# 0xPolygonZero/plonky2

Measured on NVIDIA H100. Metric: goldilocks_field_elements_per_s_ntt_lde_merkle, higher is better.
Workload: dtype u64

## Files before the change

plonky2_b200/csrc/gl_lazy.cuh:

```cuda
#pragma once
#include "gl_field.cuh"

namespace gl {

struct L3 {
    uint32_t w0, w1;
    int32_t e;
};

GL_HD L3 l3_from(uint64_t x) { return L3{(uint32_t)x, (uint32_t)(x >> 32), 0}; }

#if defined(__CUDA_ARCH__)
__device__ __forceinline__ L3 l3_add(L3 a, L3 b) {
    L3 r;
    asm("add.cc.u32 %0, %3, %6;\n\taddc.cc.u32 %1, %4, %7;\n\taddc.u32 %2, %5, %8;"
        : "=r"(r.w0), "=r"(r.w1), "=r"(r.e)
        : "r"(a.w0), "r"(a.w1), "r"(a.e), "r"(b.w0), "r"(b.w1), "r"(b.e));
    return r;
}
__device__ __forceinline__ L3 l3_sub(L3 a, L3 b) {
    L3 r;
    asm("sub.cc.u32 %0, %3, %6;\n\tsubc.cc.u32 %1, %4, %7;\n\tsubc.u32 %2, %5, %8;"
        : "=r"(r.w0), "=r"(r.w1), "=r"(r.e)
        : "r"(a.w0), "r"(a.w1), "r"(a.e), "r"(b.w0), "r"(b.w1), "r"(b.e));
    return r;
}
template <int S>
__device__ __forceinline__ L3 l3_shift(L3 a) {
    static_assert(S >= 0 && S < 96, "shift out of range");
    if constexpr (S == 0) return a;
    constexpr int q = S / 32, r = S % 32;
    uint32_t c0, c1, c2;
    int32_t c3;
    if constexpr (r == 0) {
        c0 = a.w0;
        c1 = a.w1;
        c2 = (uint32_t)a.e;
        c3 = a.e >> 31;
    } else {
        c0 = a.w0 << r;
        c1 = __funnelshift_l(a.w0, a.w1, r);
        c2 = __funnelshift_l(a.w1, (uint32_t)a.e, r);
        c3 = a.e >> (32 - r);
    }
    const int32_t s3 = c3 >> 31;
    L3 o;
    if (q == 0) {
        uint32_t t0, t1, b1, be;
        asm("add.cc.u32 %0, %2, %3;\n\taddc.u32 %1, %4, 0;" : "=r"(t0), "=r"(t1) : "r"(c2), "r"((uint32_t)c3), "r"((uint32_t)s3));
        asm("add.cc.u32 %0, %2, %3;\n\taddc.u32 %1, 0, 0;" : "=r"(b1), "=r"(be) : "r"(c1), "r"(c2));
        asm("sub.cc.u32 %0, %3, %5;\n\tsubc.cc.u32 %1, %4, %6;\n\tsubc.u32 %2, %7, %8;"
            : "=r"(o.w0), "=r"(o.w1), "=r"(o.e)
            : "r"(c0), "r"(b1), "r"(t0), "r"(t1), "r"(be), "r"((int32_t)t1 >> 31));
    } else if (q == 1) {
        uint32_t b1, be, t0, t1;
        int32_t t2;
        asm("add.cc.u32 %0, %2, %3;\n\taddc.u32 %1, 0, 0;" : "=r"(b1), "=r"(be) : "r"(c0), "r"(c1));
        asm("add.cc.u32 %0, %3, %4;\n\taddc.cc.u32 %1, %5, 0;\n\taddc.u32 %2, %6, 0;"
            : "=r"(t0), "=r"(t1), "=r"(t2)
            : "r"(c1), "r"(c2), "r"((uint32_t)c3), "r"(s3));
        asm("sub.cc.u32 %0, 0, %3;\n\tsubc.cc.u32 %1, %4, %5;\n\tsubc.u32 %2, %6, %7;"
            : "=r"(o.w0), "=r"(o.w1), "=r"(o.e)
            : "r"(t0), "r"(b1), "r"(t1), "r"(be), "r"(t2));
    } else {
        uint32_t u0, u1, v0, v1, t1;
        int32_t t2;
        asm("add.cc.u32 %0, %2, %3;\n\taddc.u32 %1, 0, 0;" : "=r"(u0), "=r"(u1) : "r"(c0), "r"(c1));
        asm("sub.cc.u32 %0, %0, %2;\n\tsubc.u32 %1, %1, %3;" : "+r"(u0), "+r"(u1) : "r"((uint32_t)c3), "r"((uint32_t)s3));
        asm("add.cc.u32 %0, %2, %3;\n\taddc.u32 %1, %4, 0;" : "=r"(v0), "=r"(v1) : "r"(c2), "r"((uint32_t)c3), "r"((uint32_t)s3));
        asm("add.cc.u32 %0, %2, %3;\n\taddc.u32 %1, %4, %5;" : "=r"(t1), "=r"(t2) : "r"(u1), "r"(v0), "r"((int32_t)u1 >> 31), "r"(v1));
        asm("sub.cc.u32 %0, 0, %3;\n\tsubc.cc.u32 %1, %4, %5;\n\tsubc.u32 %2, 0, %6;"
            : "=r"(o.w0), "=r"(o.w1), "=r"(o.e)
            : "r"(u0), "r"(c0), "r"(t1), "r"(t2));
    }
    return o;
}
__device__ __forceinline__ uint64_t l3_norm(L3 a) {
    uint32_t w0, w1, e;
    asm("add.cc.u32 %0, %3, 0x00100000;\n\taddc.cc.u32 %1, %4, 0xfff00000;\n\taddc.u32 %2, %5, 0x000fffff;"
        : "=r"(w0), "=r"(w1), "=r"(e)
        : "r"(a.w0), "r"(a.w1), "r"(a.e));
    return reduce96(pack64(w0, w1), e);
}
#else
inline __int128 l3_val(L3 a) { return (__int128)a.w0 + ((__int128)a.w1 << 32) + (__int128)a.e * ((__int128)1 << 64); }
inline L3 l3_of(__int128 v) {
    L3 r;
    r.w0 = (uint32_t)(unsigned __int128)v;
    r.w1 = (uint32_t)((unsigned __int128)v >> 32);
    r.e = (int32_t)(v >> 64);
    return r;
}
inline L3 l3_add(L3 a, L3 b) { return l3_of(l3_val(a) + l3_val(b)); }
inline L3 l3_sub(L3 a, L3 b) { return l3_of(l3_val(a) - l3_val(b)); }
inline uint64_t l3_norm(L3 a) {
    __int128 v = l3_val(a) % (__int128)P;
    if (v < 0) v += P;
    return (uint64_t)v;
}
template <int S>
inline L3 l3_shift(L3 a) { return l3_from(mul_pow2(l3_norm(a), (uint32_t)S)); }
#endif

template <int S>
GL_HD L3 l3_shift_c(L3 a) { return l3_shift<S>(a); }
template <int M, int L, int B>
struct DftLazyBfly {
    static GL_HD void run(L3* r) {
        constexpr int half = 1 << (M - 1 - L);
        constexpr int j = B % half, blk = (B / half) * 2 * half;
        constexpr int sh = (96 / half) * j;
        const L3 u = r[blk + j], v = r[blk + j + half];
        r[blk + j] = l3_add(u, v);
        r[blk + j + half] = l3_shift_c<sh>(l3_sub(u, v));
        if constexpr (B + 1 < (1 << (M - 1))) DftLazyBfly<M, L, B + 1>::run(r);
        else if constexpr (L + 1 < M) DftLazyBfly<M, L + 1, 0>::run(r);
    }
};
template <int M>
GL_HD void dft_lazy(L3* r) {
    if constexpr (M > 0) DftLazyBfly<M, 0, 0>::run(r);
}

}
```

plonky2_b200/csrc/gl_ntt.cuh:

```cuda
#pragma once
#include "gl_lazy.cuh"

namespace gl {

constexpr int NTT_MAX_LOG_PASS = 10;
constexpr int NTT_COL_MIN_LOG = 5;

GL_HD constexpr int ntt_r2(int log) { return log / 2; }
GL_HD constexpr int ntt_r1(int log) { return log - log / 2; }

template <int LOG>
struct PassCfg {
    static constexpr int R1 = ntt_r1(LOG), R2 = ntt_r2(LOG);
    static constexpr int E = 1 << R1, TPT = 1 << R2, NSUB = E / TPT;
    static constexpr int ROW_THREADS = (TPT * 8 < 32) ? 32 : TPT * 8;
    static constexpr int LPC = ROW_THREADS / TPT;
    static constexpr int ROW_MIN_BLOCKS = (E >= 32 ? 512 : 768) / ROW_THREADS;
    static constexpr int ROW_PITCH = TPT + 1;
    static constexpr int ROW_S_WORDS = E * ROW_PITCH;
    static constexpr int GATHER_PITCH = (1 << LOG) + 2;
    static constexpr int T = (256 / TPT) < 8 ? 8 : (256 / TPT);
    static constexpr int COL_THREADS = T * TPT;
    static constexpr int COL_MIN_BLOCKS = (E >= 32 ? 512 : 768) / COL_THREADS;
    static constexpr int COL_QPITCH = TPT * T + 8;
    static constexpr int COL_S_WORDS = E * COL_QPITCH;
};
GL_HD constexpr size_t ntt_row_smem_bytes(int log, bool natural) {
    const int r1 = ntt_r1(log), r2 = ntt_r2(log), E = 1 << r1, TPT = 1 << r2;
    const int threads = (TPT * 8 < 32) ? 32 : TPT * 8, lpc = threads / TPT;
    const size_t s = (size_t)lpc * E * (TPT + 1), g = natural ? (size_t)lpc * ((1 << log) + 2) : 0;
    return (s > g ? s : g) * 8;
}
GL_HD constexpr size_t ntt_col_smem_bytes(int log) {
    const int r1 = ntt_r1(log), r2 = ntt_r2(log), E = 1 << r1, TPT = 1 << r2;
    const int T = (256 / TPT) < 8 ? 8 : (256 / TPT);
    return (size_t)E * (TPT * T + 8) * 8;
}

GL_HD uint64_t table_step_entry(int log, uint32_t idx, uint64_t scale, uint64_t base) {
    const int r1 = ntt_r1(log), r2 = ntt_r2(log);
    const uint32_t t = idx & ((1u << r2) - 1), q = idx >> r2;
    const uint64_t k = bitrev32(q, (uint32_t)r1);
    uint64_t v = pow(root_of_unity((uint32_t)log), k * t);
    if (base != 1) v = mul(v, pow(base, t));
    if (scale != 1) v = mul(v, scale);
    return v;
}
GL_HD uint64_t table_post_entry(int a, int b, size_t idx, uint64_t base) {
    const size_t p = idx >> b, j2 = idx & (((size_t)1 << b) - 1);
    const uint64_t k1 = bitrev32((uint32_t)p, (uint32_t)a);
    uint64_t v = pow(root_of_unity((uint32_t)(a + b)), k1 * j2);
    if (base != 1) v = mul(v, pow(base, j2));
    return v;
}

template <int LOG>
GL_HD void pass_step1(uint64_t* x, const uint64_t* tw, const uint64_t* uq, bool tw_full, int t) {
    using Cf = PassCfg<LOG>;
    L3 r[Cf::E];
#pragma unroll
    for (int q = 0; q < Cf::E; q++) {
        uint64_t v = x[q];
        if (uq && q) v = mul(v, uq[q]);
        r[q] = l3_from(v);
    }
    dft_lazy<Cf::R1>(r);
#pragma unroll
    for (int q = 0; q < Cf::E; q++) {
        uint64_t y = l3_norm(r[q]);
        if (Cf::R2 > 0 && (q || tw_full)) y = mul(y, tw[q * Cf::TPT + t]);
        if (Cf::R2 == 0 && tw_full) y = mul(y, tw[0]);
        x[q] = y;
    }
}
template <int LOG>
GL_HD void pass_step2(uint64_t* z) {
    using Cf = PassCfg<LOG>;
    L3 r[Cf::TPT];
#pragma unroll
    for (int j = 0; j < Cf::TPT; j++) r[j] = l3_from(z[j]);
    dft_lazy<Cf::R2>(r);
#pragma unroll
    for (int j = 0; j < Cf::TPT; j++) z[j] = l3_norm(r[j]);
}

struct ColPass {
    const uint64_t* in;
    uint64_t* out;
    size_t in_stride, out_stride;
    const uint64_t* tw;
    const uint64_t* twa;
    int log_c;
    int log_rb;
    int tw_full;
    int has_uq;
    uint64_t uq[32];
};
template <int LOG>
GL_HD void col_unit(const ColPass& cp, int blk, size_t& in_off, size_t& out_off, int& tile) {
    using Cf = PassCfg<LOG>;
    const int tiles = (1 << cp.log_c) / Cf::T;
    tile = blk % tiles;
    const int unit = blk / tiles;
    const size_t rb = (size_t)unit & (((size_t)1 << cp.log_rb) - 1), col = (size_t)unit >> cp.log_rb;
    const size_t blk_words = (size_t)1 << (LOG + cp.log_c);
    in_off = col * cp.in_stride + rb * blk_words;
    out_off = col * cp.out_stride + rb * blk_words;
}
template <int LOG>
GL_HD void col_load(const ColPass& cp, int blk, int tid, uint64_t* x) {
    using Cf = PassCfg<LOG>;
    const int tt = tid % Cf::T, t = tid / Cf::T;
    size_t in_off, out_off;
    int tile;
    col_unit<LOG>(cp, blk, in_off, out_off, tile);
    const size_t C = (size_t)1 << cp.log_c;
    const uint64_t* src = cp.in + in_off + (size_t)tile * Cf::T + tt;
#pragma unroll
    for (int q = 0; q < Cf::E; q++) x[q] = src[(size_t)(t + Cf::TPT * q) * C];
}
template <int LOG>
GL_HD void col_phase1(const ColPass& cp, uint64_t* S, int blk, int tid, uint64_t* x) {
    using Cf = PassCfg<LOG>;
    const int tt = tid % Cf::T, t = tid / Cf::T;
    size_t in_off, out_off;
    int tile;
    col_unit<LOG>(cp, blk, in_off, out_off, tile);
    const size_t C = (size_t)1 << cp.log_c;
    pass_step1<LOG>(x, cp.tw, cp.has_uq ? cp.uq : nullptr, cp.tw_full != 0, t);
    if (Cf::R2 == 0) {
        uint64_t* dst = cp.out + out_off + (size_t)tile * Cf::T + tt;
        const uint64_t* twa = cp.twa + (size_t)tile * Cf::T + tt;
#pragma unroll
        for (int q = 0; q < Cf::E; q++) dst[(size_t)q * C] = mul(x[q], twa[(size_t)q * C]);
        return;
    }
#pragma unroll
    for (int q = 0; q < Cf::E; q++) S[q * Cf::COL_QPITCH + t * Cf::T + tt] = x[q];
}
template <int LOG>
GL_HD void col_phase2_load(const uint64_t* S, int tid, uint64_t* z ) {
    using Cf = PassCfg<LOG>;
    const int tt = tid % Cf::T, t = tid / Cf::T;
#pragma unroll
    for (int m = 0; m < Cf::NSUB; m++) {
        const int q = t + Cf::TPT * m;
#pragma unroll
        for (int j = 0; j < Cf::TPT; j++) z[m * Cf::TPT + j] = S[q * Cf::COL_QPITCH + j * Cf::T + tt];
    }
}
template <int LOG>
GL_HD void col_phase2_dft(uint64_t* z) {
    using Cf = PassCfg<LOG>;
#pragma unroll
    for (int m = 0; m < Cf::NSUB; m++) pass_step2<LOG>(z + m * Cf::TPT);
}
template <int LOG>
GL_HD int col_twiddle_slot(int tid, int i) { return i * PassCfg<LOG>::COL_THREADS + tid; }
template <int LOG>
GL_HD const uint64_t* col_twiddle_src(const ColPass& cp, int blk, int tid, int i) {
    using Cf = PassCfg<LOG>;
    const int tt = tid % Cf::T, t = tid / Cf::T;
    size_t in_off, out_off;
    int tile;
    col_unit<LOG>(cp, blk, in_off, out_off, tile);
    const int m = i / Cf::TPT, j = i % Cf::TPT;
    const size_t p = (size_t)(t + Cf::TPT * m) * Cf::TPT + j;
    return cp.twa + (p << cp.log_c) + (size_t)tile * Cf::T + tt;
}
template <int LOG>
GL_HD void col_phase2_store(const ColPass& cp, int blk, int tid, const uint64_t* z, const uint64_t* tws, size_t stride_j,
                            size_t stride_m) {
    using Cf = PassCfg<LOG>;
    const int tt = tid % Cf::T, t = tid / Cf::T;
    size_t in_off, out_off;
    int tile;
    col_unit<LOG>(cp, blk, in_off, out_off, tile);
    const size_t C = (size_t)1 << cp.log_c;
    uint64_t* dst = cp.out + out_off + (size_t)tile * Cf::T + tt;
#pragma unroll
    for (int m = 0; m < Cf::NSUB; m++) {
#pragma unroll
        for (int j = 0; j < Cf::TPT; j++) {
            const int i = m * Cf::TPT + j;
            const size_t p = (size_t)(t + Cf::TPT * m) * Cf::TPT + j;
            dst[p * C] = mul(z[i], tws[m * stride_m + j * stride_j]);
        }
    }
}
template <int LOG>
GL_HD void col_phase2(const ColPass& cp, const uint64_t* S, int blk, int tid) {
    using Cf = PassCfg<LOG>;
    if (Cf::R2 == 0) return;
    uint64_t z[Cf::E];
    col_phase2_load<LOG>(S, tid, z);
    col_phase2_dft<LOG>(z);
    const size_t C = (size_t)1 << cp.log_c;
    col_phase2_store<LOG>(cp, blk, tid, z, col_twiddle_src<LOG>(cp, blk, tid, 0), C, (size_t)Cf::TPT * Cf::TPT * C);
}

enum RowMode { RM_BITREV = 0, RM_NATURAL = 1 };
struct RowPass {
    const uint64_t* in;
    uint64_t* out;
    size_t in_stride, out_stride;
    const uint64_t* tw;
    int log_r;
    int ncols;
    int tw_full;
    int has_uq;
    int reverse;
    size_t row0;
    int n_peer;
    uint64_t* out_peer[7];
    uint64_t uq[32];
};
template <int LOG, int MODE>
GL_HD bool row_line(const RowPass& rp, int blk, int l, size_t& col, size_t& prow, size_t& kbase) {
    using Cf = PassCfg<LOG>;
    const size_t L = (size_t)blk * Cf::LPC + l;
    const size_t R = (size_t)1 << rp.log_r;
    col = L >> rp.log_r;
    const size_t low = L & (R - 1);
    if (MODE == RM_BITREV) {
        prow = low;
        kbase = 0;
    } else {
        kbase = low;
        prow = rp.log_r ? (size_t)bitrev32((uint32_t)low, (uint32_t)rp.log_r) : 0;
    }
    return col < (size_t)rp.ncols;
}
template <int LOG>
GL_HD int row_blocks(const RowPass& rp) {
    using Cf = PassCfg<LOG>;
    const size_t lines = (size_t)rp.ncols << rp.log_r;
    return (int)((lines + Cf::LPC - 1) / Cf::LPC);
}
template <int LOG, int MODE>
GL_HD void row_load(const RowPass& rp, int blk, int tid, uint64_t* x) {
    using Cf = PassCfg<LOG>;
    const int l = tid / Cf::TPT, t = tid % Cf::TPT;
    size_t col, prow, kbase;
    const bool live = row_line<LOG, MODE>(rp, blk, l, col, prow, kbase);
    const uint64_t* src = rp.in + col * rp.in_stride + (prow << LOG) + t;
#pragma unroll
    for (int q = 0; q < Cf::E; q++) x[q] = live ? src[Cf::TPT * q] : 0;
}
template <int LOG, int MODE>
GL_HD void row_phase1(const RowPass& rp, uint64_t* S, int blk, int tid, uint64_t* x) {
    using Cf = PassCfg<LOG>;
    const int l = tid / Cf::TPT, t = tid % Cf::TPT;
    pass_step1<LOG>(x, rp.tw, rp.has_uq ? rp.uq : nullptr, rp.tw_full != 0, t);
    if (Cf::R2 == 0) return;
    uint64_t* Sl = S + (size_t)l * Cf::ROW_S_WORDS;
#pragma unroll
    for (int q = 0; q < Cf::E; q++) Sl[q * Cf::ROW_PITCH + t] = x[q];
}
template <int LOG>
GL_HD uint32_t row_natural_index(int q, int j) {
    using Cf = PassCfg<LOG>;
    return bitrev32((uint32_t)q, Cf::R1) + (uint32_t)Cf::E * (Cf::R2 ? bitrev32((uint32_t)j, Cf::R2) : 0u);
}
template <int LOG>
GL_HD void row_phase2_load(const uint64_t* S, int tid, int m, uint64_t* z) {
    using Cf = PassCfg<LOG>;
    const int l = tid / Cf::TPT, t = tid % Cf::TPT;
    const uint64_t* Sl = S + (size_t)l * Cf::ROW_S_WORDS;
    const int q = t + Cf::TPT * m;
#pragma unroll
    for (int j = 0; j < Cf::TPT; j++) z[j] = Sl[q * Cf::ROW_PITCH + j];
}
template <int LOG>
GL_HD void row_store_bitrev(const RowPass& rp, int blk, int tid, int m, const uint64_t* z) {
    using Cf = PassCfg<LOG>;
    const int l = tid / Cf::TPT, t = tid % Cf::TPT;
    size_t col, prow, kbase;
    if (!row_line<LOG, RM_BITREV>(rp, blk, l, col, prow, kbase)) return;
    uint64_t* dst = rp.out + col * rp.out_stride + rp.row0 + (prow << LOG);
    if constexpr (Cf::R2 == 0) {
#pragma unroll
        for (int q = 0; q < Cf::E; q++) dst[q] = canon(z[q]);
    } else {
        const int q = t + Cf::TPT * m;
        uint64_t* d = dst + (size_t)q * Cf::TPT;
#if defined(__CUDA_ARCH__)
#pragma unroll
        for (int j = 0; j < Cf::TPT; j += 2) {
            ulonglong2 v;
            v.x = canon(z[j]);
            v.y = canon(z[j + 1]);
            *reinterpret_cast<ulonglong2*>(d + j) = v;
        }
#else
        for (int j = 0; j < Cf::TPT; j++) d[j] = canon(z[j]);
#endif
    }
}
template <int LOG>
GL_HD void row_gather_write(uint64_t* G, int tid, int m, const uint64_t* z) {
    using Cf = PassCfg<LOG>;
    const int l = tid / Cf::TPT, t = tid % Cf::TPT;
    uint64_t* Gl = G + (size_t)l * Cf::GATHER_PITCH;
    if (Cf::R2 == 0) {
#pragma unroll
        for (int q = 0; q < Cf::E; q++) Gl[row_natural_index<LOG>(q, 0)] = canon(z[q]);
        return;
    }
    const int q = t + Cf::TPT * m;
#pragma unroll
    for (int j = 0; j < Cf::TPT; j++) Gl[row_natural_index<LOG>(q, j)] = canon(z[j]);
}
template <int LOG>
GL_HD void row_store_natural(const RowPass& rp, const uint64_t* G, int blk, int tid, int nthreads) {
    using Cf = PassCfg<LOG>;
    const size_t R = (size_t)1 << rp.log_r, n = R << LOG;
    for (int e = tid; e < Cf::LPC * (1 << LOG); e += nthreads) {
        int l, k2;
        if (rp.log_r) {
            l = e % Cf::LPC;
            k2 = e / Cf::LPC;
        } else {
            k2 = e & ((1 << LOG) - 1);
            l = e >> LOG;
        }
        size_t col, prow, kbase;
        if (!row_line<LOG, RM_NATURAL>(rp, blk, l, col, prow, kbase)) continue;
        size_t k = kbase + ((size_t)k2 << rp.log_r);
        if (rp.reverse) k = (n - k) & (n - 1);
        const uint64_t v = G[(size_t)l * Cf::GATHER_PITCH + k2];
        const size_t at = col * rp.out_stride + k;
        rp.out[at] = v;
        for (int p = 0; p < rp.n_peer; p++) rp.out_peer[p][at] = v;
    }
}

struct NttPlan {
    int a1, a2, b;
};
GL_HD NttPlan ntt_plan(int log_n) {
    NttPlan p{0, 0, log_n};
    if (log_n <= NTT_MAX_LOG_PASS) return p;
    if (log_n <= 2 * NTT_MAX_LOG_PASS) {
        p.b = (log_n + 1) / 2;
        p.a1 = log_n - p.b;
        return p;
    }
    p.b = (log_n + 2) / 3;
    p.a2 = (log_n - p.b + 1) / 2;
    p.a1 = log_n - p.b - p.a2;
    return p;
}


struct TableReq {
    int a, b;
    uint64_t scale, base;
};
struct NttJob {
    NttPlan pl;
    ColPass c1, c2;
    RowPass rp;
    TableReq c1_step, c1_post, c2_step, c2_post, row_step;
};
inline void ntt_make_job(int log_n, NttPlan pl, uint64_t scale, uint64_t shift, NttJob& job) {
    job = NttJob{};
    job.pl = pl;
    const bool coset = canon(shift) != 1;
    const uint64_t one = 1;
    RowPass& rp = job.rp;
    rp.log_r = log_n - pl.b;
    auto fill_uq = [](uint64_t* uq, int log_pass, uint64_t sq) {
        const int E = 1 << ntt_r1(log_pass);
        uint64_t acc = 1;
        for (int q = 0; q < E; q++, acc = mul(acc, sq)) uq[q] = canon(acc);
    };
    if (pl.a1 == 0) {
        job.row_step = TableReq{pl.b, 0, scale, coset ? shift : one};
        rp.tw_full = (canon(scale) != 1 || coset) ? 1 : 0;
        rp.has_uq = coset ? 1 : 0;
        if (coset) fill_uq(rp.uq, pl.b, pow(shift, (uint64_t)1 << ntt_r2(pl.b)));
        return;
    }
    const int c1_log = log_n - pl.a1;
    ColPass& c1 = job.c1;
    c1.log_c = c1_log;
    c1.log_rb = 0;
    job.c1_step = TableReq{pl.a1, 0, one, coset ? pow(shift, (uint64_t)1 << c1_log) : one};
    job.c1_post = TableReq{pl.a1, c1_log, one, coset ? shift : one};
    c1.tw_full = coset ? 1 : 0;
    c1.has_uq = coset ? 1 : 0;
    if (coset) fill_uq(c1.uq, pl.a1, pow(shift, ((uint64_t)1 << ntt_r2(pl.a1)) << c1_log));
    if (pl.a2) {
        ColPass& c2 = job.c2;
        c2.log_c = pl.b;
        c2.log_rb = pl.a1;
        job.c2_step = TableReq{pl.a2, 0, one, one};
        job.c2_post = TableReq{pl.a2, pl.b, one, one};
    }
    job.row_step = TableReq{pl.b, 0, scale, one};
    rp.tw_full = canon(scale) != 1 ? 1 : 0;
}
template <int LOG>
GL_HD int col_blocks(const ColPass& cp, size_t ncols) {
    return (int)((ncols << cp.log_rb) * (((size_t)1 << cp.log_c) / PassCfg<LOG>::T));
}

}
```

plonky2_b200/csrc/gl_ntt_host.cuh:

```cuda
#pragma once

template <int LOG, bool ASYNC_TW>
__global__ void __launch_bounds__(PassCfg<LOG>::COL_THREADS, PassCfg<LOG>::COL_MIN_BLOCKS) k_ntt_col(ColPass cp) {
    using Cf = PassCfg<LOG>;
    extern __shared__ __align__(16) u64 smem[];
    u64* tw_s = smem;
    u64* S = smem + (1 << LOG);
    u64* mbar = S + Cf::COL_S_WORDS;
    tma_table_issue(tw_s, cp.tw, (uint32_t)((1 << LOG) * 8), mbar);
    u64 x[Cf::E];
    col_load<LOG>(cp, blockIdx.x, threadIdx.x, x);
    __syncthreads();
    ColPass c2 = cp;
    c2.tw = tw_s;
    tma_table_wait(mbar);
    col_phase1<LOG>(c2, S, blockIdx.x, threadIdx.x, x);
    if (Cf::R2 == 0) return;
    __syncthreads();
    if (!ASYNC_TW) {
        col_phase2<LOG>(c2, S, blockIdx.x, threadIdx.x);
        return;
    }
    col_phase2_load<LOG>(S, threadIdx.x, x);
    __syncthreads();
#pragma unroll
    for (int i = 0; i < Cf::E; i++) {
        const u64* src = col_twiddle_src<LOG>(cp, blockIdx.x, threadIdx.x, i);
        asm volatile("cp.async.ca.shared.global [%0], [%1], 8;" ::"r"(smem_u32(S + col_twiddle_slot<LOG>(threadIdx.x, i))), "l"(src)
                     : "memory");
    }
    asm volatile("cp.async.commit_group;" ::: "memory");
    col_phase2_dft<LOG>(x);
    asm volatile("cp.async.wait_group 0;" ::: "memory");
    col_phase2_store<LOG>(cp, blockIdx.x, threadIdx.x, x, S + col_twiddle_slot<LOG>(threadIdx.x, 0), Cf::COL_THREADS,
                          (size_t)Cf::TPT * Cf::COL_THREADS);
}

template <int LOG, bool ASYNC_TW>
__global__ void __launch_bounds__(PassCfg<LOG>::COL_THREADS, PassCfg<LOG>::COL_MIN_BLOCKS) k_ntt_col_shared(ColPass cp) {
    using Cf = PassCfg<LOG>;
    static_assert(Cf::E == Cf::TPT, "shared-body column pass needs an even LOG");
    extern __shared__ __align__(16) u64 smem[];
    u64* tw_s = smem;
    u64* S = smem + (1 << LOG);
    u64* mbar = S + Cf::COL_S_WORDS;
    tma_table_issue(tw_s, cp.tw, (uint32_t)((1 << LOG) * 8), mbar);
    u64 x[Cf::E];
    col_load<LOG>(cp, blockIdx.x, threadIdx.x, x);
    __syncthreads();
    tma_table_wait(mbar);
    const int tt = threadIdx.x % Cf::T, t = threadIdx.x / Cf::T;
    size_t in_off, out_off;
    int tile;
    col_unit<LOG>(cp, blockIdx.x, in_off, out_off, tile);
    const size_t C = (size_t)1 << cp.log_c;
    if (cp.has_uq) {
#pragma unroll
        for (int q = 1; q < Cf::E; q++) x[q] = mul(x[q], cp.uq[q]);
    }
    const u64* twp = tw_s + t;
    size_t tws = Cf::TPT;
    bool skip0 = cp.tw_full == 0;
#pragma unroll 1
    for (int s = 0; s < 2; s++) {
        L3 r[Cf::E];
#pragma unroll
        for (int q = 0; q < Cf::E; q++) r[q] = l3_from(x[q]);
        dft_lazy<Cf::R1>(r);
        if (ASYNC_TW && s == 1) asm volatile("cp.async.wait_group 0;" ::: "memory");
#pragma unroll
        for (int q = 0; q < Cf::E; q++) {
            u64 y = l3_norm(r[q]);
            if (!(q == 0 && skip0)) y = mul(y, twp[(size_t)q * tws]);
            x[q] = y;
        }
        if (s == 0) {
#pragma unroll
            for (int q = 0; q < Cf::E; q++) S[q * Cf::COL_QPITCH + t * Cf::T + tt] = x[q];
            __syncthreads();
#pragma unroll
            for (int j = 0; j < Cf::TPT; j++) x[j] = S[t * Cf::COL_QPITCH + j * Cf::T + tt];
            skip0 = false;
            const u64* tw2 = cp.twa + (((size_t)t * Cf::TPT) << cp.log_c) + (size_t)tile * Cf::T + tt;
            if (ASYNC_TW) {
                __syncthreads();
#pragma unroll
                for (int j = 0; j < Cf::TPT; j++)
                    asm volatile("cp.async.ca.shared.global [%0], [%1], 8;" ::"r"(smem_u32(S + col_twiddle_slot<LOG>(threadIdx.x, j))),
                                 "l"(tw2 + (size_t)j * C)
                                 : "memory");
                asm volatile("cp.async.commit_group;" ::: "memory");
                twp = S + col_twiddle_slot<LOG>(threadIdx.x, 0);
                tws = Cf::COL_THREADS;
            } else {
                twp = tw2;
                tws = C;
            }
        }
    }
    u64* dst = cp.out + out_off + (size_t)tile * Cf::T + tt;
#pragma unroll
    for (int j = 0; j < Cf::TPT; j++) dst[((size_t)t * Cf::TPT + j) * C] = x[j];
}

template <int LOG, int MODE>
__global__ void __launch_bounds__(PassCfg<LOG>::ROW_THREADS, PassCfg<LOG>::ROW_MIN_BLOCKS) k_ntt_row(RowPass rp) {
    using Cf = PassCfg<LOG>;
    extern __shared__ __align__(16) u64 smem[];
    u64* tw_s = smem;
    u64* S = smem + (1 << LOG);
    u64* mbar = S + ntt_row_smem_bytes(LOG, MODE == RM_NATURAL) / 8;
    RowPass r2 = rp;
    u64 x[Cf::E];
    if (Cf::R2 > 0 && LOG >= 4) {
        tma_table_issue(tw_s, rp.tw, (uint32_t)((1 << LOG) * 8), mbar);
        row_load<LOG, MODE>(rp, blockIdx.x, threadIdx.x, x);
        __syncthreads();
        r2.tw = tw_s;
        tma_table_wait(mbar);
    } else {
        row_load<LOG, MODE>(rp, blockIdx.x, threadIdx.x, x);
    }
    row_phase1<LOG, MODE>(r2, S, blockIdx.x, threadIdx.x, x);
    if (Cf::R2 == 0) {
        if (MODE == RM_BITREV) {
            row_store_bitrev<LOG>(r2, blockIdx.x, threadIdx.x, 0, x);
        } else {
            row_gather_write<LOG>(S, threadIdx.x, 0, x);
            __syncthreads();
            row_store_natural<LOG>(r2, S, blockIdx.x, threadIdx.x, blockDim.x);
        }
        return;
    }
    __syncwarp();
    if (MODE == RM_BITREV) {
#pragma unroll
        for (int m = 0; m < Cf::NSUB; m++) {
            u64 z[Cf::TPT];
            row_phase2_load<LOG>(S, threadIdx.x, m, z);
            pass_step2<LOG>(z);
            row_store_bitrev<LOG>(r2, blockIdx.x, threadIdx.x, m, z);
        }
    } else {
        u64 z[Cf::NSUB][Cf::TPT];
#pragma unroll
        for (int m = 0; m < Cf::NSUB; m++) {
            row_phase2_load<LOG>(S, threadIdx.x, m, z[m]);
            pass_step2<LOG>(z[m]);
        }
        __syncthreads();
#pragma unroll
        for (int m = 0; m < Cf::NSUB; m++) row_gather_write<LOG>(S, threadIdx.x, m, z[m]);
        __syncthreads();
        row_store_natural<LOG>(r2, S, blockIdx.x, threadIdx.x, blockDim.x);
    }
}

template <int LOG, int MODE>
__global__ void __launch_bounds__(PassCfg<LOG>::ROW_THREADS, PassCfg<LOG>::ROW_MIN_BLOCKS) k_ntt_row_shared(RowPass rp) {
    using Cf = PassCfg<LOG>;
    static_assert(Cf::E == Cf::TPT && Cf::R2 > 0 && LOG >= 4, "shared-body row pass needs an even LOG >= 4");
    extern __shared__ __align__(16) u64 smem[];
    u64* tw_s = smem;
    u64* S = smem + (1 << LOG);
    u64* mbar = S + ntt_row_smem_bytes(LOG, MODE == RM_NATURAL) / 8;
    u64 x[Cf::E];
    tma_table_issue(tw_s, rp.tw, (uint32_t)((1 << LOG) * 8), mbar);
    row_load<LOG, MODE>(rp, blockIdx.x, threadIdx.x, x);
    __syncthreads();
    tma_table_wait(mbar);
    const int l = threadIdx.x / Cf::TPT, t = threadIdx.x % Cf::TPT;
    u64* Sl = S + (size_t)l * Cf::ROW_S_WORDS;
    if (rp.has_uq) {
#pragma unroll
        for (int q = 1; q < Cf::E; q++) x[q] = mul(x[q], rp.uq[q]);
    }
    const bool skip0 = rp.tw_full == 0;
    bool do_mul = true;
#pragma unroll 1
    for (int s = 0; s < 2; s++) {
        L3 r[Cf::E];
#pragma unroll
        for (int q = 0; q < Cf::E; q++) r[q] = l3_from(x[q]);
        dft_lazy<Cf::R1>(r);
#pragma unroll
        for (int q = 0; q < Cf::E; q++) {
            u64 y = l3_norm(r[q]);
            if (do_mul && !(q == 0 && skip0)) y = mul(y, tw_s[q * Cf::TPT + t]);
            x[q] = y;
        }
        if (s == 0) {
#pragma unroll
            for (int q = 0; q < Cf::E; q++) Sl[q * Cf::ROW_PITCH + t] = x[q];
            __syncwarp();
#pragma unroll
            for (int j = 0; j < Cf::TPT; j++) x[j] = Sl[t * Cf::ROW_PITCH + j];
            do_mul = false;
        }
    }
    if (MODE == RM_BITREV) {
        row_store_bitrev<LOG>(rp, blockIdx.x, threadIdx.x, 0, x);
    } else {
        __syncthreads();
        row_gather_write<LOG>(S, threadIdx.x, 0, x);
        __syncthreads();
        row_store_natural<LOG>(rp, S, blockIdx.x, threadIdx.x, blockDim.x);
    }
}

__global__ void k_fill_step(int log, u64 scale, u64 base, u64* out) {
    uint32_t j = blockIdx.x * blockDim.x + threadIdx.x;
    if (j < (1u << log)) out[j] = table_step_entry(log, j, scale, base);
}
__global__ void k_fill_post(int a, int b, u64 base, u64* out) {
    size_t i = (size_t)blockIdx.x * blockDim.x + threadIdx.x;
    if (i < ((size_t)1 << (a + b))) out[i] = table_post_entry(a, b, i, base);
}
__global__ void k_fill_pows(const u64* bases, int ntab, size_t count, u64* out) {
    size_t i = (size_t)blockIdx.x * blockDim.x + threadIdx.x;
    if (i >= count * ntab) return;
    size_t t = i / count, e = i % count;
    out[i] = gl::pow(bases[t], e);
}
__global__ void k_mul_pows(u64* data, size_t stride, size_t n, const u64* hi, const u64* lo, int lowbits) {
    size_t k = (size_t)blockIdx.x * blockDim.x + threadIdx.x;
    if (k >= n) return;
    u64* col = data + (size_t)blockIdx.y * stride;
    u64 f = mul(hi[k >> lowbits], lo[k & (((size_t)1 << lowbits) - 1)]);
    col[k] = canon(mul(col[k], f));
}

template <int LOG>
static int launch_col(gl_ctx* ctx, const ColPass& cp, size_t ncols) {
    const int nblocks = col_blocks<LOG>(cp, ncols);
    const size_t smem = ((size_t)(1 << LOG) + PassCfg<LOG>::COL_S_WORDS) * 8 + 16;
    auto go = [&](auto kern) -> int {
        const void* fn = (const void*)kern;
        if (!ctx->smem_attr_done.count(fn)) {
            CK(ctx, cudaFuncSetAttribute(kern, cudaFuncAttributeMaxDynamicSharedMemorySize, (int)smem));
            CK(ctx, cudaFuncSetAttribute(kern, cudaFuncAttributePreferredSharedMemoryCarveout, cudaSharedmemCarveoutMaxShared));
            ctx->smem_attr_done.insert(fn);
        }
        kern<<<nblocks, PassCfg<LOG>::COL_THREADS, smem, ctx->stream>>>(cp);
        CKL(ctx);
        return GL_OK;
    };
    if constexpr (PassCfg<LOG>::E == PassCfg<LOG>::TPT) {
        if (ctx->ntt_variant == 0) return cp.has_uq ? go(k_ntt_col_shared<LOG, true>) : go(k_ntt_col_shared<LOG, false>);
    }
    return cp.has_uq ? go(k_ntt_col<LOG, true>) : go(k_ntt_col<LOG, false>);
}
template <int LOG, int MODE>
static int launch_row(gl_ctx* ctx, const RowPass& rp) {
    const size_t smem = (size_t)(1 << LOG) * 8 + ntt_row_smem_bytes(LOG, MODE == RM_NATURAL) + 16;
    auto go = [&](auto kern) -> int {
        const void* fn = (const void*)kern;
        if (!ctx->smem_attr_done.count(fn)) {
            CK(ctx, cudaFuncSetAttribute(kern, cudaFuncAttributeMaxDynamicSharedMemorySize, (int)smem));
            CK(ctx, cudaFuncSetAttribute(kern, cudaFuncAttributePreferredSharedMemoryCarveout, cudaSharedmemCarveoutMaxShared));
            ctx->smem_attr_done.insert(fn);
        }
        kern<<<row_blocks<LOG>(rp), PassCfg<LOG>::ROW_THREADS, smem, ctx->stream>>>(rp);
        CKL(ctx);
        return GL_OK;
    };
    if constexpr (PassCfg<LOG>::E == PassCfg<LOG>::TPT && LOG >= 4) {
        if (ctx->ntt_variant == 0) return go(k_ntt_row_shared<LOG, MODE>);
    }
    return go(k_ntt_row<LOG, MODE>);
}
static int dispatch_col(gl_ctx* ctx, int a, const ColPass& cp, size_t ncols) {
    switch (a) {
        case 5: return launch_col<5>(ctx, cp, ncols);
        case 6: return launch_col<6>(ctx, cp, ncols);
        case 7: return launch_col<7>(ctx, cp, ncols);
        case 8: return launch_col<8>(ctx, cp, ncols);
        case 9: return launch_col<9>(ctx, cp, ncols);
        case 10: return launch_col<10>(ctx, cp, ncols);
    }
    return set_err(ctx, GL_ERR_UNSUPPORTED, "column pass log %d", a);
}
static int dispatch_row(gl_ctx* ctx, int b, int mode, const RowPass& rp) {
#define ROW_CASE(L)                                                     \
    case L:                                                             \
        return mode == RM_BITREV ? launch_row<L, RM_BITREV>(ctx, rp) : launch_row<L, RM_NATURAL>(ctx, rp);
    switch (b) {
        ROW_CASE(1) ROW_CASE(2) ROW_CASE(3) ROW_CASE(4) ROW_CASE(5) ROW_CASE(6) ROW_CASE(7) ROW_CASE(8) ROW_CASE(9) ROW_CASE(10)
    }
#undef ROW_CASE
    return set_err(ctx, GL_ERR_UNSUPPORTED, "row pass log %d", b);
}

static void table_cache_trim(gl_ctx* ctx, size_t incoming_bytes) {
    const size_t cap = (size_t)3 << 30;
    if (ctx->table_bytes + incoming_bytes <= cap) return;
    for (auto& kv : ctx->step_tabs) cudaFreeAsync(kv.second, ctx->stream);
    for (auto& kv : ctx->post_tabs) cudaFreeAsync(kv.second, ctx->stream);
    ctx->step_tabs.clear();
    ctx->post_tabs.clear();
    ctx->table_bytes = 0;
}
static int get_step(gl_ctx* ctx, int log, u64 scale, u64 base, const u64** out) {
    auto key = std::make_tuple(log, canon(scale), canon(base));
    auto it = ctx->step_tabs.find(key);
    if (it == ctx->step_tabs.end()) {
        const size_t words = ((size_t)1 << log) < 2 ? 2 : ((size_t)1 << log);
        DevBuf p(ctx);
        TRY(p.alloc(words));
        k_fill_step<<<((1 << log) + 255) / 256, 256, 0, ctx->stream>>>(log, canon(scale), canon(base), p.get());
        CKL(ctx);
        ctx->table_bytes += words * 8;
        it = ctx->step_tabs.emplace(key, p.release()).first;
    }
    *out = it->second;
    return GL_OK;
}
static int get_post(gl_ctx* ctx, int a, int b, u64 base, const u64** out) {
    auto key = std::make_tuple(a, b, canon(base));
    auto it = ctx->post_tabs.find(key);
    if (it == ctx->post_tabs.end()) {
        const size_t words = (size_t)1 << (a + b);
        DevBuf p(ctx);
        TRY(p.alloc(words));
        k_fill_post<<<(unsigned)((words + 255) / 256), 256, 0, ctx->stream>>>(a, b, canon(base), p.get());
        CKL(ctx);
        ctx->table_bytes += words * 8;
        it = ctx->post_tabs.emplace(key, p.release()).first;
    }
    *out = it->second;
    return GL_OK;
}
static uint32_t group_cols(const gl_ctx* ctx, int log_n, uint32_t ncols) {
    uint32_t g = ctx->ntt_group;
    if (g == 0) {
        size_t col_bytes = (size_t)8 << log_n;
        size_t target = (size_t)1 << 30;
        g = (uint32_t)(target / col_bytes);
        if (g < 8) g = 8;
    }
    g = (g + 7) & ~7u;
    if (g > ((ncols + 7) & ~7u)) g = (ncols + 7) & ~7u;
    return g;
}

static int build_pow_tables(gl_ctx* ctx, const std::vector<u64>& bases, size_t count, DevBuf& out) {
    const int ntab = (int)bases.size();
    DevBuf dbases(ctx);
    TRY(dbases.alloc(ntab));
    TRY(h2d(ctx, dbases.get(), bases.data(), ntab));
    TRY(out.alloc(count * ntab));
    size_t total = count * ntab;
    k_fill_pows<<<(unsigned)((total + 255) / 256), 256, 0, ctx->stream>>>(dbases.get(), ntab, count, out.get());
    CKL(ctx);
    return GL_OK;
}

struct PeerOuts {
    int n = 0;
    u64* p[7] = {nullptr, nullptr, nullptr, nullptr, nullptr, nullptr, nullptr};
};
static int ntt_forward(gl_ctx* ctx, const u64* in, size_t in_stride, u64* out, size_t out_stride, size_t row0, int log_n,
                       uint32_t ncols, int mode, bool reverse, u64 scale, u64 shift, const PeerOuts* peers = nullptr) {
    if (ncols == 0) return GL_OK;
    if (log_n < 1 || log_n > 3 * NTT_MAX_LOG_PASS) return set_err(ctx, GL_ERR_UNSUPPORTED, "log_n %d not in 1..30", log_n);
    const NttPlan pl = ntt_plan(log_n);
    const size_t n = (size_t)1 << log_n;
    table_cache_trim(ctx, 2 * n * 8 + (1 << 16));
    NttJob job;
    ntt_make_job(log_n, pl, scale, shift, job);
    RowPass& rp = job.rp;
    rp.out_stride = out_stride;
    rp.reverse = reverse ? 1 : 0;
    rp.row0 = row0;
    rp.n_peer = peers ? peers->n : 0;
    for (int i = 0; i < rp.n_peer; i++) rp.out_peer[i] = peers->p[i];
    TRY(get_step(ctx, job.row_step.a, job.row_step.scale, job.row_step.base, &rp.tw));
    if (pl.a1 == 0) {
        rp.in = in;
        rp.in_stride = in_stride;
        rp.out = out;
        rp.ncols = (int)ncols;
        return dispatch_row(ctx, pl.b, mode, rp);
    }
    const uint32_t G = group_cols(ctx, log_n, ncols);
    TRY(ensure_scratch(ctx, (size_t)G * n));
    ColPass &c1 = job.c1, &c2 = job.c2;
    c1.out = ctx->scratch;
    c1.in_stride = in_stride;
    c1.out_stride = n;
    TRY(get_step(ctx, job.c1_step.a, job.c1_step.scale, job.c1_step.base, &c1.tw));
    TRY(get_post(ctx, job.c1_post.a, job.c1_post.b, job.c1_post.base, &c1.twa));
    if (pl.a2) {
        c2.in = c2.out = ctx->scratch;
        c2.in_stride = c2.out_stride = n;
        TRY(get_step(ctx, job.c2_step.a, job.c2_step.scale, job.c2_step.base, &c2.tw));
        TRY(get_post(ctx, job.c2_post.a, job.c2_post.b, job.c2_post.base, &c2.twa));
    }
    rp.in = ctx->scratch;
    rp.in_stride = n;
    for (uint32_t g0 = 0; g0 < ncols; g0 += G) {
        const uint32_t gc = (ncols - g0 < G) ? ncols - g0 : G;
        c1.in = in + (size_t)g0 * in_stride;
        TRY(dispatch_col(ctx, pl.a1, c1, gc));
        if (pl.a2) TRY(dispatch_col(ctx, pl.a2, c2, gc));
        rp.out = out + (size_t)g0 * out_stride;
        for (int i = 0; i < rp.n_peer; i++) rp.out_peer[i] = peers->p[i] + (size_t)g0 * out_stride;
        rp.ncols = (int)gc;
        TRY(dispatch_row(ctx, pl.b, mode, rp));
    }
    return GL_OK;
}

__global__ void k_scale1(u64* data, size_t stride, uint32_t ncols, u64 f) {
    uint32_t b = blockIdx.x * blockDim.x + threadIdx.x;
    if (b < ncols) data[(size_t)b * stride] = canon(mul(data[(size_t)b * stride], f));
}

static int ntt_natural(gl_ctx* ctx, const u64* in, size_t in_stride, u64* out, size_t out_stride, int log_n,
                       uint32_t ncols, bool inverse, u64 shift, const PeerOuts* peers = nullptr) {
    if (ncols == 0) return GL_OK;
    const size_t n = (size_t)1 << log_n;
    if (peers && peers->n && (log_n == 0 || canon(shift) != 1))
        return set_err(ctx, GL_ERR_UNSUPPORTED, "multi-destination transforms need log_n >= 1 and no coset shift");
    if (log_n == 0) {
        if (in != out)
            CK(ctx, cudaMemcpy2DAsync(out, out_stride * 8, in, in_stride * 8, 8, ncols, cudaMemcpyDeviceToDevice,
                                      ctx->stream));
        k_scale1<<<(ncols + 127) / 128, 128, 0, ctx->stream>>>(out, out_stride, ncols, 1);
        CKL(ctx);
        return GL_OK;
    }
    if (!inverse) return ntt_forward(ctx, in, in_stride, out, out_stride, 0, log_n, ncols, RM_NATURAL, false, 1, shift, peers);
    TRY(ntt_forward(ctx, in, in_stride, out, out_stride, 0, log_n, ncols, RM_NATURAL, true, inverse_2exp((uint32_t)log_n), 1,
                    peers));
    if (canon(shift) != 1) {
        const int lowbits = log_n > 12 ? 12 : log_n;
        const size_t lo_cnt = (size_t)1 << lowbits, hi_cnt = (size_t)1 << (log_n - lowbits);
        const u64 sinv = gl::inv(shift);
        const size_t tcnt = lo_cnt > hi_cnt ? lo_cnt : hi_cnt;
        DevBuf tabs(ctx);
        TRY(build_pow_tables(ctx, std::vector<u64>{gl::pow(sinv, lo_cnt), sinv}, tcnt, tabs));
        for (uint32_t b0 = 0; b0 < ncols; b0 += MAX_GRID_Y) {
            const uint32_t bc = (ncols - b0 < MAX_GRID_Y) ? ncols - b0 : MAX_GRID_Y;
            k_mul_pows<<<dim3((unsigned)((n + 255) / 256), bc), 256, 0, ctx->stream>>>(
                out + (size_t)b0 * out_stride, out_stride, n, tabs.get(), tabs.get() + tcnt, lowbits);
            CKL(ctx);
        }
    }
    return GL_OK;
}

__global__ void k_lde_const(const u64* coeffs, size_t stride, uint32_t ncols, int ncos, u64* lde, size_t lde_stride) {
    uint32_t i = blockIdx.x * blockDim.x + threadIdx.x;
    if (i >= ncols * (uint32_t)ncos) return;
    uint32_t col = i / ncos, c = i % ncos;
    lde[(size_t)col * lde_stride + c] = canon(coeffs[(size_t)col * stride]);
}

static int lde_columns(gl_ctx* ctx, const u64* coeffs, size_t coeff_stride, uint32_t ncols, int log_n, int rate_bits,
                       u64 base_shift, u64* lde, size_t lde_stride) {
    if (ncols == 0) return GL_OK;
    const size_t n = (size_t)1 << log_n;
    const int ncos = 1 << rate_bits;
    if (log_n == 0) {
        k_lde_const<<<(ncols * ncos + 127) / 128, 128, 0, ctx->stream>>>(coeffs, coeff_stride, ncols, ncos, lde, lde_stride);
        CKL(ctx);
        return GL_OK;
    }
    const u64 wN = root_of_unity((uint32_t)(log_n + rate_bits));
    const uint32_t G = log_n > NTT_MAX_LOG_PASS ? group_cols(ctx, log_n, ncols) : ncols;
    for (uint32_t g0 = 0; g0 < ncols; g0 += G) {
        const uint32_t gc = (ncols - g0 < G) ? ncols - g0 : G;
        for (int c = 0; c < ncos; c++) {
            const u64 s = mul(base_shift, gl::pow(wN, bitrev32((uint32_t)c, (uint32_t)rate_bits)));
            TRY(ntt_forward(ctx, coeffs + (size_t)g0 * coeff_stride, coeff_stride, lde + (size_t)g0 * lde_stride, lde_stride,
                            (size_t)c * n, log_n, gc, RM_BITREV, false, 1, s));
        }
    }
    return GL_OK;
}
```

Before: 7.782 billion.

## Fuse prescale mults into lazy DFT, cheaper l3_norm, tiled bitrev row stores

Replaces the l3_norm reduction with a shorter carry-based sequence that avoids reduce96. Adds l3_mul, which produces a lazy 96-bit product without full reduction, and uses it to fold the uq prescale multiply into the DFT input conversion in the column and step passes. The bit-reversed row store now stages results through shared memory so global writes are coalesced. This adds smem traffic and warp syncs, and relies on the lazy representation staying in range.

```diff
diff --git a/plonky2_b200/csrc/gl_lazy.cuh b/plonky2_b200/csrc/gl_lazy.cuh
--- a/plonky2_b200/csrc/gl_lazy.cuh
+++ b/plonky2_b200/csrc/gl_lazy.cuh
@@ -76,11 +76,33 @@
     return o;
 }
 __device__ __forceinline__ uint64_t l3_norm(L3 a) {
-    uint32_t w0, w1, e;
-    asm("add.cc.u32 %0, %3, 0x00100000;\n\taddc.cc.u32 %1, %4, 0xfff00000;\n\taddc.u32 %2, %5, 0x000fffff;"
-        : "=r"(w0), "=r"(w1), "=r"(e)
+    uint32_t r0, r1;
+    asm("{\n\t.reg .u32 s, t0, t1, d;\n\t"
+        "shr.s32 s, %4, 31;\n\t"
+        "sub.cc.u32 t0, 0, %4;\n\t"
+        "subc.u32 t1, %4, s;\n\t"
+        "add.cc.u32 %0, %2, t0;\n\t"
+        "addc.cc.u32 %1, %3, t1;\n\t"
+        "addc.u32 d, s, 0;\n\t"
+        "neg.s32 t0, d;\n\t"
+        "shr.s32 t1, d, 31;\n\t"
+        "add.cc.u32 %0, %0, t0;\n\t"
+        "addc.u32 %1, %1, t1;\n\t}"
+        : "=&r"(r0), "=&r"(r1)
         : "r"(a.w0), "r"(a.w1), "r"(a.e));
-    return reduce96(pack64(w0, w1), e);
+    return pack64(r0, r1);
+}
+__device__ __forceinline__ L3 l3_mul(uint64_t a, uint64_t b) {
+    uint64_t lo, hi;
+    mul_wide(a, b, lo, hi);
+    uint32_t t0, t1, b1, be;
+    L3 o;
+    asm("add.cc.u32 %0, %2, %3;\n\taddc.u32 %1, 0, 0;" : "=r"(t0), "=r"(t1) : "r"(lo32(hi)), "r"(hi32(hi)));
+    asm("add.cc.u32 %0, %2, %3;\n\taddc.u32 %1, 0, 0;" : "=r"(b1), "=r"(be) : "r"(hi32(lo)), "r"(lo32(hi)));
+    asm("sub.cc.u32 %0, %3, %5;\n\tsubc.cc.u32 %1, %4, %6;\n\tsubc.u32 %2, %7, 0;"
+        : "=r"(o.w0), "=r"(o.w1), "=r"(o.e)
+        : "r"(lo32(lo)), "r"(b1), "r"(t0), "r"(t1), "r"(be));
+    return o;
 }
 #else
 inline __int128 l3_val(L3 a) { return (__int128)a.w0 + ((__int128)a.w1 << 32) + (__int128)a.e * ((__int128)1 << 64); }
@@ -100,6 +122,7 @@
 }
 template <int S>
 inline L3 l3_shift(L3 a) { return l3_from(mul_pow2(l3_norm(a), (uint32_t)S)); }
+inline L3 l3_mul(uint64_t a, uint64_t b) { return l3_from(mul(a, b)); }
 #endif
 
 template <int S>
diff --git a/plonky2_b200/csrc/gl_ntt.cuh b/plonky2_b200/csrc/gl_ntt.cuh
--- a/plonky2_b200/csrc/gl_ntt.cuh
+++ b/plonky2_b200/csrc/gl_ntt.cuh
@@ -59,11 +59,7 @@
     using Cf = PassCfg<LOG>;
     L3 r[Cf::E];
 #pragma unroll
-    for (int q = 0; q < Cf::E; q++) {
-        uint64_t v = x[q];
-        if (uq && q) v = mul(v, uq[q]);
-        r[q] = l3_from(v);
-    }
+    for (int q = 0; q < Cf::E; q++) r[q] = (uq && q) ? l3_mul(x[q], uq[q]) : l3_from(x[q]);
     dft_lazy<Cf::R1>(r);
 #pragma unroll
     for (int q = 0; q < Cf::E; q++) {
@@ -296,6 +292,26 @@
         for (int j = 0; j < Cf::TPT; j++) d[j] = canon(z[j]);
 #endif
     }
+}
+template <int LOG>
+GL_HD void row_bitrev_tile_write(uint64_t* S, int tid, const uint64_t* z) {
+    using Cf = PassCfg<LOG>;
+    static_assert(Cf::E == Cf::TPT, "transposed bit-reversed stores need E == TPT");
+    const int l = tid / Cf::TPT, t = tid % Cf::TPT;
+    uint64_t* Sl = S + (size_t)l * Cf::ROW_S_WORDS;
+#pragma unroll
+    for (int j = 0; j < Cf::TPT; j++) Sl[t * Cf::ROW_PITCH + j] = canon(z[j]);
+}
+template <int LOG>
+GL_HD void row_store_bitrev_tile(const RowPass& rp, const uint64_t* S, int blk, int tid) {
+    using Cf = PassCfg<LOG>;
+    const int l = tid / Cf::TPT, t = tid % Cf::TPT;
+    size_t col, prow, kbase;
+    if (!row_line<LOG, RM_BITREV>(rp, blk, l, col, prow, kbase)) return;
+    const uint64_t* Sl = S + (size_t)l * Cf::ROW_S_WORDS;
+    uint64_t* dst = rp.out + col * rp.out_stride + rp.row0 + (prow << LOG) + t;
+#pragma unroll
+    for (int k = 0; k < Cf::E; k++) dst[k * Cf::TPT] = Sl[k * Cf::ROW_PITCH + t];
 }
 template <int LOG>
 GL_HD void row_gather_write(uint64_t* G, int tid, int m, const uint64_t* z) {
diff --git a/plonky2_b200/csrc/gl_ntt_host.cuh b/plonky2_b200/csrc/gl_ntt_host.cuh
--- a/plonky2_b200/csrc/gl_ntt_host.cuh
+++ b/plonky2_b200/csrc/gl_ntt_host.cuh
@@ -54,10 +54,11 @@
     int tile;
     col_unit<LOG>(cp, blockIdx.x, in_off, out_off, tile);
     const size_t C = (size_t)1 << cp.log_c;
-    if (cp.has_uq) {
+    if (!ASYNC_TW && cp.has_uq) {
 #pragma unroll
         for (int q = 1; q < Cf::E; q++) x[q] = mul(x[q], cp.uq[q]);
     }
+    bool prescale = ASYNC_TW && cp.has_uq;
     const u64* twp = tw_s + t;
     size_t tws = Cf::TPT;
     bool skip0 = cp.tw_full == 0;
@@ -65,7 +66,8 @@
     for (int s = 0; s < 2; s++) {
         L3 r[Cf::E];
 #pragma unroll
-        for (int q = 0; q < Cf::E; q++) r[q] = l3_from(x[q]);
+        for (int q = 0; q < Cf::E; q++) r[q] = (prescale && q) ? l3_mul(x[q], cp.uq[q]) : l3_from(x[q]);
+        prescale = false;
         dft_lazy<Cf::R1>(r);
         if (ASYNC_TW && s == 1) asm volatile("cp.async.wait_group 0;" ::: "memory");
 #pragma unroll
@@ -199,7 +201,10 @@
         }
     }
     if (MODE == RM_BITREV) {
-        row_store_bitrev<LOG>(rp, blockIdx.x, threadIdx.x, 0, x);
+        __syncwarp();
+        row_bitrev_tile_write<LOG>(S, threadIdx.x, x);
+        __syncwarp();
+        row_store_bitrev_tile<LOG>(rp, S, blockIdx.x, threadIdx.x);
     } else {
         __syncthreads();
         row_gather_write<LOG>(S, threadIdx.x, 0, x);
```

New measurement: 8.154 billion (median of 6 runs). 4.8% higher.
